# Aleph-Alpha/magma

Measured on NVIDIA H100. Metric: image-caption samples/sec (fwd+bwd), higher is better.
Workload: dtype bf16

## Files before the change

include/magma_b200.h:

```cpp
#ifndef MAGMA_B200_H_
#define MAGMA_B200_H_

#include <stddef.h>
#include <stdint.h>

#ifdef __cplusplus
extern "C" {
#endif

#define MB200_VERSION 100

enum {
  MB200_OK = 0,
  MB200_E_SHAPE = -1,
  MB200_E_DTYPE = -2,
  MB200_E_ALIGN = -3,
  MB200_E_ARCH = -4,
  MB200_E_CUDA = -5,
  MB200_E_NCCL = -6,
  MB200_E_ARG = -7
};

enum { MB200_BF16 = 0, MB200_F32 = 1 };

enum {
  MB200_ACT_NONE = 0,
  MB200_ACT_GELU_NEW = 1,
  MB200_ACT_QUICK_GELU = 2,
  MB200_ACT_RELU = 3,
  MB200_ACT_RELU_POST = 4
};
enum {
  MB200_DACT_NONE = 0,
  MB200_DACT_GELU_NEW = 1,
  MB200_DACT_RELU = 3
};

int mb200_version(void);
const char* mb200_last_error(void);
int mb200_check_device(void);
int mb200_set_gemm_sm_limit(int n_sms);
int mb200_set_optimizer_grid(int n_blocks);
long long mb200_launch_count(void);
int mb200_prof_enable(int on);
int mb200_prof_read(double* gemm_ms, double* gemm_flops, double* gemm_bytes, long long* gemm_launches);

typedef struct {
  const void* ptr;
  int64_t ld;
  int64_t bs0, bs1;
  int32_t mn_major;
  int32_t static_data;
} mb200_operand;

typedef struct {
  int32_t M, N, K;
  int32_t nb0, nb1;
  int32_t c_dtype;
  mb200_operand A, B;
  void* C;
  int64_t ldc, c_bs0, c_bs1;
  float alpha;
  int32_t act;
  int32_t dact;
  int32_t accumulate;
  const void* bias;
  void* aux_out;
  const void* aux_in;
  const void* res1;
  const void* res2;
  int64_t ld_res;
  int32_t force_bn;
  int32_t generic_epilogue;
  int32_t rope_mode;
  const void* rope_tab;
  int32_t rope_S, rope_hd, rope_rot, rope_ncols;
  void* splitk_ws;
  int64_t splitk_ws_bytes;
} mb200_gemm_args;

int mb200_gemm(const mb200_gemm_args* args, void* stream);


int mb200_layernorm_fwd(const void* x, int64_t ldx, const void* gamma, const void* beta, void* y, int64_t ldy,
                        float* mean, float* rstd, int32_t rows, int32_t d, float eps, void* stream);
int mb200_layernorm_bwd(const void* dy, int64_t lddy, const void* x, int64_t ldx, const void* gamma,
                        const float* mean, const float* rstd, const void* res, int64_t ldres, void* dx, int64_t lddx,
                        int32_t rows, int32_t d, void* stream);
int mb200_layernorm_param_grad(const void* dy, int64_t lddy, const void* x, int64_t ldx, const float* mean,
                               const float* rstd, float* dgamma, float* dbeta, int32_t rows, int32_t d,
                               int32_t accumulate, void* stream);
int mb200_layernorm_param_grad_rows(const void* dy, int64_t lddy, const void* x, int64_t ldx, const float* mean,
                                    const float* rstd, float* dgamma, float* dbeta, int32_t rows, int32_t d,
                                    int32_t accumulate, void* stream);
int mb200_rope(void* qkv, int64_t ld, int32_t rows, int32_t S, int32_t H, int32_t hd, int32_t rot, int32_t pos0,
               int32_t inverse, void* stream);
int mb200_rope_table(float* tab, int32_t S, int32_t rot, int32_t pos0, void* stream);
int mb200_softmax_fwd(const float* s, int64_t lds, int64_t s_bs, void* p, int64_t ldp, int64_t p_bs, int32_t nz,
                      int32_t Sq, int32_t Sk, float scale, int32_t causal, int32_t koff, void* stream);
int mb200_softmax_bwd(const float* dp, int64_t lddp, int64_t dp_bs, const void* p, int64_t ldp, int64_t p_bs,
                      void* ds, int64_t ldds, int64_t ds_bs, int32_t nz, int32_t Sq, int32_t Sk, float scale,
                      void* stream);
int mb200_build_labels(const int64_t* captions, int64_t ldc, int64_t* labels, int32_t B, int32_t S, int32_t L,
                       int64_t eos, void* stream);
int mb200_embed_assemble(const int64_t* captions, int64_t ldc, const void* wte, const void* prefix, int32_t L,
                         void* x, int32_t B, int32_t S, int32_t d, int32_t vocab, void* stream);
int mb200_embed_gather(const int64_t* ids, const void* wte, void* out, int32_t n, int32_t d, int32_t vocab,
                       void* stream);
int mb200_cross_entropy(const void* logits, int64_t ldv, const int64_t* labels, int32_t B, int32_t S, int32_t V,
                        float* row_loss, int32_t* n_valid, float* loss, void* dlogits, float grad_scale,
                        void* stream);
int mb200_colsum(const void* x, int64_t ldx, int32_t rows, int32_t cols, float* out, int32_t accumulate,
                 void* stream);
int mb200_dropout_fwd(const void* x, void* y, uint8_t* mask, int64_t n, float p, uint64_t seed, void* stream);
int mb200_dropout_apply(const void* x, const uint8_t* mask, void* y, int64_t n, float p, void* stream);
int mb200_patchify(const void* img, void* patches, int64_t ldp, int32_t B, int32_t R, int32_t P, void* stream);
int mb200_vit_assemble(void* x, const void* pe, const void* cls, const void* pos, int32_t B, int32_t T, int32_t w,
                       void* stream);
int mb200_nchw_to_nhwc8(const void* src, void* dst, int32_t B, int32_t C, int32_t H, int32_t W, void* stream);
int mb200_im2col3x3(const void* src, void* dst, int32_t B, int32_t H, int32_t W, int32_t C, int32_t stride,
                    void* stream);
int mb200_avgpool_nhwc(const void* src, void* dst, int32_t B, int32_t H, int32_t W, int32_t C, int32_t k, void* stream);
int mb200_col_moments(const void* u, int64_t ldu, const void* v, int64_t ldv, const void* mask, int64_t ldm, int32_t rows,
                      int32_t cols, float* out1, float* out2, void* stream);
int mb200_channel_affine(const void* x1, const float* a1, const void* x2, const float* a2, const float* c0,
                         const void* mask, const void* res, int32_t relu, void* y, int64_t rows, int32_t C, void* stream);
int mb200_bn_finalize_fwd(const float* s1, const float* s2, const float* gamma, const float* beta, int64_t rows, float eps,
                          float momentum, float* running_mean, float* running_var, float* mean, float* rstd, float* scale,
                          float* shift, int32_t C, void* stream);
int mb200_bn_bwd_coeffs(const float* s1, const float* t, const float* mean, const float* rstd, const float* gamma,
                        int64_t rows, float* dgamma, float* dbeta, int32_t accumulate, float* A, float* Bc, float* Cc,
                        int32_t C, void* stream);
int mb200_col2im3x3(const void* dcols, void* dx, int32_t B, int32_t H, int32_t W, int32_t C, int32_t stride, void* stream);
int mb200_avgpool_nhwc_bwd(const void* dy, void* dx, int32_t B, int32_t H, int32_t W, int32_t C, int32_t k, void* stream);
int mb200_argmax(const void* x, int64_t ldx, int32_t rows, int32_t V, int64_t* out, void* stream);
int mb200_sample(const void* logits, int32_t dtype, int64_t ld, int32_t rows, int32_t V, float temperature,
                 int32_t top_k, float top_p, uint64_t seed, uint64_t offset, int64_t* tokens, uint8_t* keep_mask,
                 void* stream);
int mb200_add(const void* a, const void* b, const void* c, void* y, int64_t n, void* stream);
int mb200_peer_reduce_bcast(void* const* bufs, int32_t world, int64_t offset, int64_t n, int32_t max_blocks,
                            void* stream);

int mb200_sumsq(const float* x, int64_t n, float* out, void* stream);
int mb200_adamw_step(float* master, float* grad, float* exp_avg, float* exp_avg_sq, void* shadow_bf16, int64_t n,
                     float lr, float beta1, float beta2, float eps, float weight_decay, float grad_scale,
                     const float* gnorm_sq, float max_norm, int32_t step, int32_t zero_grad, void* stream);
int mb200_cast_f32_to_bf16(const float* src, void* dst, int64_t n, void* stream);
int mb200_cast_bf16_to_f32(const void* src, float* dst, int64_t n, void* stream);

enum { MB200_ADAPTER_NONE = 0, MB200_ADAPTER_NORMAL = 1, MB200_ADAPTER_PARALLEL = 2 };

typedef struct {
  const void *ln1_g, *ln1_b;
  const void* w_qkv;
  const void* b_qkv;
  const void* w_out;
  const void* b_out;
  const void *ln2_g, *ln2_b;
  const void* w_fc;
  const void* b_fc;
  const void* w_proj;
  const void* b_proj;
} mb200_vit_layer;

// ... 143 lines not shown
```

magma_b200/_lib.py:

```python
import ctypes
import os

_HERE = os.path.dirname(os.path.abspath(__file__))
LIB_PATH = os.path.join(_HERE, "lib", "libmagma_b200.so")

_lib = None


class MB200Error(RuntimeError):
    pass


class Operand(ctypes.Structure):
    _fields_ = [
        ("ptr", ctypes.c_void_p),
        ("ld", ctypes.c_int64),
        ("bs0", ctypes.c_int64),
        ("bs1", ctypes.c_int64),
        ("mn_major", ctypes.c_int32),
        ("static_data", ctypes.c_int32),
    ]


class GemmArgs(ctypes.Structure):
# ... 59 lines not shown
        (n, ctypes.c_void_p)
        for n in (
            "ln1_g", "ln1_b", "w_qkv", "b_qkv", "w_out", "b_out", "ln2_g", "ln2_b", "w_fc", "b_fc", "w_proj", "b_proj",
        )
    ]


class VitModelC(ctypes.Structure):
    _fields_ = [
        ("n_layer", ctypes.c_int32),
        ("width", ctypes.c_int32),
        ("n_head", ctypes.c_int32),
        ("patch", ctypes.c_int32),
        ("image", ctypes.c_int32),
        ("mlp", ctypes.c_int32),
        ("out_dim", ctypes.c_int32),
        ("_pad", ctypes.c_int32),
        ("w_conv", ctypes.c_void_p),
        ("ld_conv", ctypes.c_int64),
        ("cls", ctypes.c_void_p),
        ("pos", ctypes.c_void_p),
        ("ln_pre_g", ctypes.c_void_p),
        ("ln_pre_b", ctypes.c_void_p),
        ("ln_post_g", ctypes.c_void_p),
        ("ln_post_b", ctypes.c_void_p),
        ("proj_t", ctypes.c_void_p),
        ("layers", ctypes.POINTER(VitLayerC)),
    ]


class AdapterExC(ctypes.Structure):
    _fields_ = [(n, ctypes.c_void_p) for n in ("wd", "bd", "wu", "bu", "ln_g", "ln_b", "scale", "g_wd", "g_bd", "g_wu",
                                               "g_bu", "g_ln_g", "g_ln_b", "g_scale")]


class GptjLayerExC(ctypes.Structure):
    _fields_ = [
        (n, ctypes.c_void_p)
        for n in ("ln1_g", "ln1_b", "w_qkv", "w_out", "w_fc_in", "b_fc_in", "w_fc_out", "b_fc_out")
    ] + [("mlp_ad", AdapterExC), ("attn_ad", AdapterExC)]


class GptjModelExC(ctypes.Structure):
    _fields_ = [
        ("n_layer", ctypes.c_int32),
        ("d", ctypes.c_int32),
        ("n_head", ctypes.c_int32),
        ("rotary_dim", ctypes.c_int32),
        ("vocab", ctypes.c_int32),
        ("d_ff", ctypes.c_int32),
        ("mlp_adapter", ctypes.c_int32),
        ("mlp_adapter_r", ctypes.c_int32),
        ("attn_adapter", ctypes.c_int32),
        ("attn_adapter_r", ctypes.c_int32),
        ("ln_eps", ctypes.c_float),
        ("adapter_act", ctypes.c_int32),
        ("layers", ctypes.POINTER(GptjLayerExC)),
        ("lnf_g", ctypes.c_void_p),
        ("lnf_b", ctypes.c_void_p),
        ("w_lm", ctypes.c_void_p),
        ("b_lm", ctypes.c_void_p),
    ]


class VitLayerGradsC(ctypes.Structure):
    _fields_ = list(VitLayerC._fields_)


class VitGradsC(ctypes.Structure):
    _fields_ = [(n, ctypes.c_void_p) for n in ("w_conv", "cls", "pos", "ln_pre_g", "ln_pre_b", "ln_post_g",
                                               "ln_post_b", "proj")] + [("layers", ctypes.POINTER(VitLayerGradsC))]


def _setup_signatures(L):
    L.mb200_vit_workspace_bytes.restype = ctypes.c_size_t
    L.mb200_vit_train_workspace_bytes.restype = ctypes.c_size_t
    L.mb200_gptj_sched_workspace_bytes.restype = ctypes.c_size_t
    L.mb200_gptj_sched_infer_workspace_bytes.restype = ctypes.c_size_t
    L.mb200_gptj_sched_recompute_workspace_bytes.restype = ctypes.c_size_t
    L.mb200_launch_count.restype = ctypes.c_longlong


EXPORTED_SYMBOLS = [
    "mb200_version", "mb200_last_error", "mb200_check_device", "mb200_gemm",
    "mb200_launch_count", "mb200_prof_enable", "mb200_prof_read",
    "mb200_layernorm_fwd", "mb200_layernorm_bwd", "mb200_layernorm_param_grad", "mb200_rope", "mb200_rope_table",
    "mb200_softmax_fwd", "mb200_softmax_bwd", "mb200_build_labels", "mb200_embed_assemble", "mb200_embed_gather",
    "mb200_cross_entropy", "mb200_colsum", "mb200_dropout_fwd", "mb200_dropout_apply", "mb200_patchify",
    "mb200_nchw_to_nhwc8", "mb200_im2col3x3", "mb200_avgpool_nhwc",
    "mb200_vit_assemble", "mb200_argmax", "mb200_sample", "mb200_add", "mb200_peer_reduce_bcast", "mb200_sumsq", "mb200_adamw_step",
    "mb200_cast_f32_to_bf16", "mb200_cast_bf16_to_f32",
    "mb200_vit_workspace_bytes", "mb200_vit_forward", "mb200_attn_decode", "mb200_attn_fwd_tile", "mb200_attn_fwd_flash",
    "mb200_attn_bwd_tile",
    "mb200_vit_train_workspace_bytes", "mb200_vit_forward_train", "mb200_vit_backward", "mb200_quick_gelu_bwd",
    "mb200_layernorm_param_grad_rows", "mb200_set_gemm_sm_limit", "mb200_set_optimizer_grid", "mb200_scale_add", "mb200_dot",
    "mb200_gptj_sched_workspace_bytes", "mb200_gptj_sched_forward", "mb200_gptj_sched_backward",
    "mb200_col_moments", "mb200_channel_affine", "mb200_col2im3x3", "mb200_avgpool_nhwc_bwd",
    "mb200_kv_append", "mb200_gptj_sched_infer_workspace_bytes", "mb200_gptj_sched_infer",
    "mb200_gptj_sched_backward_range", "mb200_bn_finalize_fwd", "mb200_bn_bwd_coeffs",
    "mb200_gptj_sched_decode_step", "mb200_decode_embed", "mb200_decode_advance", "mb200_rope_table_dev",
    "mb200_attn_decode_dev", "mb200_gptj_sched_recompute_workspace_bytes", "mb200_gptj_sched_forward_recompute",
    "mb200_gptj_sched_backward_range_recompute",
]
```

magma_b200/csrc/gemm.cu:

```cuda
#include <mutex>
#include <stdlib.h>

#include "gemm_common.cuh"

namespace mb200 {

template <bool kOn>
struct EpiMaps {
  CUtensorMap m[3];
};
template <>
struct EpiMaps<false> {};

template <int BN, bool A_MN, bool B_MN, bool EPI_TMA, uint32_t FORM = EF_RUNTIME>
__global__ void __launch_bounds__(kThreads, 1)
gemm_wgmma_kernel(const __grid_constant__ CUtensorMap tmA, const __grid_constant__ CUtensorMap tmB,
                  const __grid_constant__ EpiMaps<EPI_TMA> tmE, const __grid_constant__ GemmKernelParams p) {
  using C_ = Cfg<BN>;
  constexpr int kStages = C_::kStages;

  extern __shared__ uint8_t smem_raw[];
  uint8_t* smem = smem_raw + ((1024u - (smem_u32(smem_raw) & 1023u)) & 1023u);
  uint8_t* smem_a = smem;
  uint8_t* smem_b = smem + kStages * C_::kABytes;
// ... 171 lines not shown
  cuuint32_t estr[4] = {1, 1, 1, 1};
  if (!op.mn_major) {
    dims[0] = (cuuint64_t)K;
    dims[1] = (cuuint64_t)rows;
    box[0] = BK;
    box[1] = (cuuint32_t)box_rows;
  } else {
    dims[0] = (cuuint64_t)rows;
    dims[1] = (cuuint64_t)K;
    box[0] = 64;
    box[1] = BK;
  }
  dims[2] = (cuuint64_t)nb0;
  dims[3] = (cuuint64_t)nb1;
  box[2] = 1;
  box[3] = 1;
  strides[0] = (cuuint64_t)op.ld * 2;
  strides[1] = (cuuint64_t)(nb0 > 1 ? op.bs0 : op.ld) * 2;
  strides[2] = (cuuint64_t)(nb1 > 1 ? op.bs1 : op.ld) * 2;
  CUresult r = enc(out, CU_TENSOR_MAP_DATA_TYPE_BFLOAT16, 4, const_cast<void*>(op.ptr), dims, strides, box, estr,
                   CU_TENSOR_MAP_INTERLEAVE_NONE, CU_TENSOR_MAP_SWIZZLE_128B, CU_TENSOR_MAP_L2_PROMOTION_L2_256B,
                   CU_TENSOR_MAP_FLOAT_OOB_FILL_NONE);
  MB_REQUIRE(r == CUDA_SUCCESS, MB200_E_CUDA,
             "cuTensorMapEncodeTiled failed (%d): dims=(%llu,%llu,%llu,%llu) strides=(%llu,%llu,%llu) box=(%u,%u)",
             (int)r, (unsigned long long)dims[0], (unsigned long long)dims[1], (unsigned long long)dims[2],
             (unsigned long long)dims[3], (unsigned long long)strides[0], (unsigned long long)strides[1],
             (unsigned long long)strides[2], box[0], box[1]);
  return 0;
}

template <int BN, bool A_MN, bool B_MN, bool EPI_TMA, uint32_t FORM = EF_RUNTIME>
static int launch_gemm(const CUtensorMap& tmA, const CUtensorMap& tmB, const EpiMaps<true>& tmE,
                       const GemmKernelParams& kp, cudaStream_t stream) {
  auto kern = gemm_wgmma_kernel<BN, A_MN, B_MN, EPI_TMA, FORM>;
  static bool attr_set = false;
  if (!attr_set) {
    MB_CUDA(cudaFuncSetAttribute(kern, cudaFuncAttributeMaxDynamicSharedMemorySize, Cfg<BN>::kSmemBytes));
    attr_set = true;
  }
  const long long items = (long long)kp.total_tiles * kp.split_k;
  int grid = items < gemm_sms() ? (int)items : gemm_sms();
  {
    const double nb = (double)kp.total_tiles / ((double)kp.tiles_m * kp.tiles_n);
    const double flops = 2.0 * kp.M * (double)kp.N * kp.K * nb;
    const double bytes = nb * (2.0 * ((double)kp.M * kp.K + (double)kp.N * kp.K) + (kp.c_f32 ? 4.0 : 2.0) * kp.M * kp.N);
    GemmProfScope prof(stream, flops, bytes);
    if constexpr (EPI_TMA)
      MB_CUDA(launch_pdl(kern, dim3(grid), dim3(kThreads), Cfg<BN>::kSmemBytes, stream, tmA, tmB, tmE, kp));
    else
      MB_CUDA(launch_pdl(kern, dim3(grid), dim3(kThreads), Cfg<BN>::kSmemBytes, stream, tmA, tmB, EpiMaps<false>{}, kp));
  }
  count_launch();
  MB_CUDA(cudaGetLastError());
  return 0;
}

template <int BN, bool EPI_TMA>
static int dispatch_major(bool a_mn, bool b_mn, const CUtensorMap& tmA, const CUtensorMap& tmB,
                          const EpiMaps<true>& tmE, const GemmKernelParams& kp, cudaStream_t s) {
  if (!a_mn && !b_mn) return launch_gemm<BN, false, false, EPI_TMA>(tmA, tmB, tmE, kp, s);
  if (!a_mn && b_mn) return launch_gemm<BN, false, true, EPI_TMA>(tmA, tmB, tmE, kp, s);
  if (a_mn && !b_mn) return launch_gemm<BN, true, false, EPI_TMA>(tmA, tmB, tmE, kp, s);
  return launch_gemm<BN, true, true, EPI_TMA>(tmA, tmB, tmE, kp, s);
}

static int dispatch_bn(int bn, bool a_mn, bool b_mn, const CUtensorMap& tmA, const CUtensorMap& tmB,
                       const EpiMaps<true>& tmE, const GemmKernelParams& kp, cudaStream_t s) {
  const bool epi = kp.epi_in != 0;
  switch (bn) {
    case 64:
      return epi ? dispatch_major<64, true>(a_mn, b_mn, tmA, tmB, tmE, kp, s)
                 : dispatch_major<64, false>(a_mn, b_mn, tmA, tmB, tmE, kp, s);
    case 128:
      return epi ? dispatch_major<128, true>(a_mn, b_mn, tmA, tmB, tmE, kp, s)
                 : dispatch_major<128, false>(a_mn, b_mn, tmA, tmB, tmE, kp, s);
    default:
      return epi ? dispatch_major<256, true>(a_mn, b_mn, tmA, tmB, tmE, kp, s)
                 : dispatch_major<256, false>(a_mn, b_mn, tmA, tmB, tmE, kp, s);
  }
}

template <uint32_t F, bool A_MN, bool B_MN>
static bool launch_form(uint32_t form, bool a_mn, bool b_mn, const CUtensorMap& tmA, const CUtensorMap& tmB,
                        const EpiMaps<true>& tmE, const GemmKernelParams& kp, cudaStream_t s, int* rc) {
  if (form != F || a_mn != A_MN || b_mn != B_MN) return false;
  *rc = launch_gemm<256, A_MN, B_MN, EpiForm<F>::kInputs != 0, F>(tmA, tmB, tmE, kp, s);
  return true;
}
static bool dispatch_form(uint32_t form, bool a_mn, bool b_mn, const CUtensorMap& tmA, const CUtensorMap& tmB,
                          const EpiMaps<true>& tmE, const GemmKernelParams& kp, cudaStream_t s, int* rc) {
#define MB_FORM(F, A_MN, B_MN) launch_form<(F), A_MN, B_MN>(form, a_mn, b_mn, tmA, tmB, tmE, kp, s, rc)
  return MB_FORM(EF_ROPE, false, false) ||
         MB_FORM(EF_RES1, false, false) ||
         MB_FORM(EF_BIAS | EF_GELU | EF_AUX_OUT, false, false) ||
         MB_FORM(EF_BIAS, false, false) ||
         MB_FORM(EF_BIAS | EF_RES1 | EF_RES2, false, false) ||
         MB_FORM(EF_DGELU, false, true) ||
         MB_FORM(0u, false, true) ||
         MB_FORM(EF_RES1, false, true) ||
         MB_FORM(EF_F32, true, true);
#undef MB_FORM
}

static uint32_t epi_form(const mb200_gemm_args* a, const GemmKernelParams& kp, int bn) {
  if (a->generic_epilogue || bn != 256) return EF_RUNTIME;
  if ((a->act != MB200_ACT_NONE && a->act != MB200_ACT_GELU_NEW) ||
      (a->dact != MB200_DACT_NONE && a->dact != MB200_DACT_GELU_NEW))
    return EF_RUNTIME;
  if (((reinterpret_cast<uintptr_t>(a->bias) | reinterpret_cast<uintptr_t>(a->aux_out)) & 7) != 0) return EF_RUNTIME;
  const uint32_t f = (a->bias ? EF_BIAS : 0u) | (kp.rope_mode ? EF_ROPE : 0u) | (a->aux_out ? EF_AUX_OUT : 0u) |
                     (a->act ? EF_GELU : 0u) | (a->dact ? EF_DGELU : 0u) | (a->res1 ? EF_RES1 : 0u) |
                     (a->res2 ? EF_RES2 : 0u) | (kp.c_f32 ? EF_F32 : 0u);
  const int inputs = (a->dact != 0) + (a->res1 != nullptr) + (a->res2 != nullptr);
  return kp.epi_in == inputs ? f : EF_RUNTIME;
}

static int make_epi_maps(EpiMaps<true>* maps, GemmKernelParams* kp, const mb200_gemm_args* a) {
  const void* ptr[3];
  long long ld[3];
  int n = 0;
  if (a->dact) {
    ptr[n] = a->aux_in;
    ld[n++] = a->ldc;
  }
  if (a->res1) {
    ptr[n] = a->res1;
    ld[n++] = a->ld_res;
  }
  if (a->res2) {
    ptr[n] = a->res2;
    ld[n++] = a->ld_res;
  }
  bool ok = (a->nb0 == 1 || a->c_bs0 % 8 == 0) && (a->nb1 == 1 || a->c_bs1 % 8 == 0);
  for (int i = 0; i < n; ++i) ok = ok && (reinterpret_cast<uintptr_t>(ptr[i]) & 15) == 0 && ld[i] % 8 == 0;
  if (n == 0 || !ok) return 0;
  for (int i = 0; i < n; ++i) {
    mb200_operand op;
    memset(&op, 0, sizeof(op));
    op.ptr = ptr[i];
    op.ld = ld[i];
    op.bs0 = a->c_bs0;
    op.bs1 = a->c_bs1;
    const int rc = make_operand_map(&maps->m[i], op, a->M, a->N, a->nb0, a->nb1, BM);
    if (rc) return rc;
  }
  kp->epi_in = n;
  return 0;
}

static int pick_bn(int M, int N, int batches) {
  if (N <= 64) return 64;
  const int tiles_m = (M + BM - 1) / BM;
  const int sms = num_sms();
  double best = 1e300;
  int best_bn = 256;
  const int cands[3] = {256, 128, 64};
  const double tile_cost[3] = {1.0, 0.55, 0.3};
  for (int i = 0; i < 3; ++i) {
    const int bn = cands[i];
    if (bn > 64 && N <= bn / 2) continue;
    const long long t = (long long)tiles_m * ((N + bn - 1) / bn) * batches;
    const long long waves = (t + sms - 1) / sms;
    const double cost = (double)waves * tile_cost[i];
    if (cost < best - 1e-12) {
      best = cost;
      best_bn = bn;
    }
  }
  return best_bn;
}

struct SmallPlan {
  int bn, split;
};
static SmallPlan plan_small_m(int N, int K, int M, size_t ws_bytes) {
  const int sms = num_sms();
  const int num_kb = (K + BK - 1) / BK;
  const double kHbmRate = 3.35e12, kItem = 4e-6, kFinalize = 4e-6;
  SmallPlan best{64, 1};
  double best_t = 1e300;
  const int cands[3] = {256, 128, 64};
  for (int i = 0; i < 3; ++i) {
    const int bn = cands[i];
    if (bn > 64 && N <= bn / 2) continue;
    const int tiles = (N + bn - 1) / bn;
    for (int split = 1; split <= 16; ++split) {
      if (split > 1) {
        if (num_kb / split < 8) break;
        if ((size_t)split * M * ((N + 3) / 4 * 4) * sizeof(float) > ws_bytes) break;
      }
      const int kb_per = (num_kb + split - 1) / split;
      const int eff_split = (num_kb + kb_per - 1) / kb_per;
      const long long items = (long long)tiles * eff_split;
      const long long waves = (items + sms - 1) / sms;
      const double active = (double)(items < sms ? items : sms);
      const double sm_rate = bn == 64 ? 40e9 : 50e9;
      const double rate = sm_rate < kHbmRate / active ? sm_rate : kHbmRate / active;
      const double t = kItem + waves * ((double)kb_per * bn * BK * 2 / rate) + (eff_split > 1 ? kFinalize : 0.0);
      if (t < best_t - 1e-12) {
        best_t = t;
        best = SmallPlan{bn, eff_split};
      }
    }
  }
  return best;
}

int gemm_impl(const mb200_gemm_args* a, cudaStream_t stream) {
  MB_REQUIRE(a != nullptr, MB200_E_ARG, "null gemm args");
  MB_REQUIRE(a->M > 0 && a->N > 0 && a->K > 0 && a->nb0 > 0 && a->nb1 > 0, MB200_E_SHAPE,
             "gemm: bad shape M=%d N=%d K=%d nb=(%d,%d)", a->M, a->N, a->K, a->nb0, a->nb1);
  MB_REQUIRE(a->c_dtype == MB200_BF16 || a->c_dtype == MB200_F32, MB200_E_DTYPE, "gemm: bad c_dtype %d", a->c_dtype);
  MB_REQUIRE(!(a->accumulate && a->c_dtype != MB200_F32), MB200_E_DTYPE, "gemm: accumulate needs f32 output");
  MB_REQUIRE(!(a->dact && !a->aux_in), MB200_E_ARG, "gemm: dact needs aux_in");
  const int celt = a->c_dtype == MB200_F32 ? 4 : 8;
  MB_REQUIRE((reinterpret_cast<uintptr_t>(a->C) & 15) == 0 && a->ldc % celt == 0, MB200_E_ALIGN,
             "gemm: C must be 16B aligned with ldc multiple of %d", celt);
  MB_REQUIRE((a->nb0 == 1 || a->c_bs0 % celt == 0) && (a->nb1 == 1 || a->c_bs1 % celt == 0), MB200_E_ALIGN,
             "gemm: C batch strides must be multiples of %d elements", celt);
  if (a->res1 || a->res2) MB_REQUIRE(a->ld_res % 8 == 0, MB200_E_ALIGN, "gemm: ld_res must be a multiple of 8");
  if (a->aux_in || a->aux_out)
    MB_REQUIRE(a->ldc % 8 == 0, MB200_E_ALIGN, "gemm: aux tensors share ldc, which must be a multiple of 8");
  int rc = check_arch();
  if (rc) return rc;

  int bn = a->force_bn ? a->force_bn : pick_bn(a->M, a->N, a->nb0 * a->nb1);
  MB_REQUIRE(bn == 64 || bn == 128 || bn == 256, MB200_E_ARG, "gemm: force_bn must be 64, 128 or 256");

  CUtensorMap tmA, tmB;
  EpiMaps<true> tmE;
  memset(&tmE, 0, sizeof(tmE));
  const bool small_m = a->M <= 32 && a->A.mn_major == 0 && a->nb0 * a->nb1 == 1 && a->c_dtype == MB200_BF16;
  int plan_split = 1;
  if (small_m && !a->force_bn) {
    const SmallPlan pl = plan_small_m(a->N, a->K, a->M, a->splitk_ws ? (size_t)a->splitk_ws_bytes : 0);
    bn = pl.bn;
    plan_split = pl.split;
  }
  rc = make_operand_map(&tmA, a->A, a->M, a->K, a->nb0, a->nb1, BM);
  if (rc) return rc;

  GemmKernelParams kp;
  memset(&kp, 0, sizeof(kp));
  kp.M = a->M;
  kp.N = a->N;
  kp.K = a->K;
  kp.nb0 = a->nb0;
  kp.tiles_m = (a->M + BM - 1) / BM;
  kp.C = a->C;
  kp.ldc = a->ldc;
  kp.c_bs0 = a->c_bs0;
  kp.c_bs1 = a->c_bs1;
  kp.alpha = a->alpha;
  kp.act = a->act;
  kp.dact = a->dact;
  kp.accumulate = a->accumulate;
  kp.bias = reinterpret_cast<const bf16*>(a->bias);
  kp.aux_out = reinterpret_cast<bf16*>(a->aux_out);
  kp.aux_in = reinterpret_cast<const bf16*>(a->aux_in);
  kp.res1 = reinterpret_cast<const bf16*>(a->res1);
  kp.res2 = reinterpret_cast<const bf16*>(a->res2);
  kp.ld_res = a->ld_res;
  kp.epi_kind = EK_GENERIC;
  kp.c_f32 = a->c_dtype == MB200_F32 ? 1 : 0;
  kp.rope_tab = reinterpret_cast<const float2*>(a->rope_tab);
  kp.rope_mode = a->rope_tab ? a->rope_mode : 0;
  kp.rope_S = a->rope_S;
  kp.rope_hd = a->rope_hd;
  kp.rope_rot = a->rope_rot;
  kp.rope_ncols = a->rope_ncols;
  if (kp.rope_mode != 0)
    MB_REQUIRE(a->rope_S > 0 && a->rope_hd > 0 && a->rope_rot % 4 == 0 && a->rope_rot <= a->rope_hd &&
                   a->rope_hd % 4 == 0 && a->rope_ncols % 4 == 0,
               MB200_E_ARG, "gemm: bad rope epilogue parameters");

  const bool amn = a->A.mn_major != 0, bmn = a->B.mn_major != 0;
  kp.split_k = 1;
  kp.kb_per_split = (a->K + BK - 1) / BK;
  const bool split_mid = !small_m && a->splitk_ws && a->M <= 128 && a->nb0 * a->nb1 == 1 && a->K >= 8192 &&
                         a->N <= 8192 && !a->force_bn;
  const int bn_few = a->N >= 256 ? 256 : (a->N > 64 ? 128 : 64);
  const int tiles_m = kp.tiles_m;
  const bool split_few = !small_m && !split_mid && a->splitk_ws && a->M > 128 && a->nb0 * a->nb1 == 1 &&
                         a->K >= 2048 && !a->force_bn && 2 * tiles_m * ((a->N + bn_few - 1) / bn_few) <= num_sms();
  if (plan_split > 1 || split_mid || split_few) {
    const int bn_s = small_m ? bn : bn_few;
    const int tiles = (a->N + bn_s - 1) / bn_s;
    const int num_kb = (a->K + BK - 1) / BK;
    int split = plan_split;
    if (split_mid || split_few) {
      split = num_sms() / (tiles * tiles_m);
      if (split > num_kb / 4) split = num_kb / 4;
    }
    const long long ld_ws = (a->N + 3) / 4 * 4;
    while (split > 1 && (size_t)split * a->M * ld_ws * sizeof(float) > (size_t)a->splitk_ws_bytes) --split;
    if (split > 1) {
      const int kb_per = (num_kb + split - 1) / split;
      split = (num_kb + kb_per - 1) / kb_per;
      bn = bn_s;
      rc = make_operand_map(&tmB, a->B, a->N, a->K, a->nb0, a->nb1, bn);
      if (rc) return rc;
      kp.tiles_n = tiles;
      kp.total_tiles = tiles_m * tiles;
      kp.split_k = split;
      kp.kb_per_split = kb_per;
      kp.splitk_ws = reinterpret_cast<float*>(a->splitk_ws);
      kp.ld_ws = ld_ws;
      GemmKernelParams kg = kp;
      kg.epi_kind = EK_SPLITK;
      rc = dispatch_bn(bn, amn, bmn, tmA, tmB, tmE, kg, stream);
      if (rc) return rc;
      const long long n4 = (long long)a->M * ((a->N + 3) / 4);
      const int fgrid = (int)((n4 + 255) / 256 > 2048 ? 2048 : (n4 + 255) / 256);
      kp.alpha = 1.f;
      MB_CUDA(launch_pdl(splitk_finalize_kernel, dim3(fgrid), dim3(256), 0, stream, kp));
      count_launch();
      return 0;
    }
  }
  rc = make_operand_map(&tmB, a->B, a->N, a->K, a->nb0, a->nb1, bn);
  if (rc) return rc;
  kp.tiles_n = (a->N + bn - 1) / bn;
  kp.total_tiles = tiles_m * kp.tiles_n * a->nb0 * a->nb1;
  rc = make_epi_maps(&tmE, &kp, a);
  if (rc) return rc;
  if (dispatch_form(epi_form(a, kp, bn), amn, bmn, tmA, tmB, tmE, kp, stream, &rc)) return rc;
  return dispatch_bn(bn, amn, bmn, tmA, tmB, tmE, kp, stream);
}

}

extern "C" int mb200_gemm(const mb200_gemm_args* args, void* stream) {
  return mb200::gemm_impl(args, reinterpret_cast<cudaStream_t>(stream));
}
```

magma_b200/csrc/gemm_common.cuh:

```cuda
#pragma once
#include <type_traits>

#include "common.cuh"

namespace mb200 {

static constexpr int BM = 128;
static constexpr int BK = 64;
static constexpr int WG_K = 16;
static constexpr int kThreads = 384;
static constexpr int kEpiCols = 64;
static constexpr int kEpiBytes = BM * kEpiCols * 4;
static constexpr int kEpiBoxBytes = BM * kEpiCols * 2;
static constexpr int kSmemBudget = 192 * 1024;

template <int BN>
struct Cfg {
  static constexpr int kABytes = BM * BK * 2;
  static constexpr int kBBytes = BN * BK * 2;
  static constexpr int kStageBytes = kABytes + kBBytes;
  static constexpr int kStagesRaw = kSmemBudget / kStageBytes;
  static constexpr int kStages = kStagesRaw > 8 ? 8 : kStagesRaw;
  static constexpr int kSmemBytes = kStages * kStageBytes + kEpiBytes + 1024  + 256 ;
  static_assert(kSmemBytes <= 227 * 1024, "GEMM shared memory exceeds the sm_90 per-block limit");
  static constexpr int kEpiBoxesPerStage = 1 + kBBytes / kEpiBoxBytes;
  static_assert(kABytes == kEpiBoxBytes && kEpiBoxesPerStage * kEpiBoxBytes <= kStageBytes, "epilogue box layout");
  static_assert(3 * (BN / kEpiCols) <= kStages * kEpiBoxesPerStage, "epilogue inputs exceed the operand ring");
};

struct GemmKernelParams {
  int M, N, K;
  int nb0;
  int tiles_m, tiles_n, total_tiles;
  void* C;
  long long ldc, c_bs0, c_bs1;
  float alpha;
  int act, dact, accumulate;
  const bf16* bias;
  bf16* aux_out;
  const bf16* aux_in;
  const bf16* res1;
  const bf16* res2;
  long long ld_res;
  int epi_in;
  const float2* rope_tab;
  int rope_mode;
  int rope_S, rope_hd, rope_rot, rope_ncols;
  int epi_kind;
  int c_f32;
  int split_k, kb_per_split;
  float* splitk_ws;
  long long ld_ws;
};

__device__ __forceinline__ float2 bf16x2_to_f32(uint32_t u) {
  return __bfloat1622float2(*reinterpret_cast<const __nv_bfloat162*>(&u));
}
__device__ __forceinline__ uint32_t f32x2_to_bf16(float a, float b) {
  __nv_bfloat162 h = __floats2bfloat162_rn(a, b);
  return *reinterpret_cast<uint32_t*>(&h);
}

template <bool kVec = false>
__device__ __forceinline__ void ld_bf16x4(const bf16* src, int n, float (&v)[4]) {
  if (kVec || (n == 4 && (reinterpret_cast<uintptr_t>(src) & 7) == 0)) {
    uint32_t u0, u1;
    asm volatile("ld.global.nc.v2.u32 {%0, %1}, [%2];" : "=r"(u0), "=r"(u1) : "l"(src));
    const float2 a = bf16x2_to_f32(u0), b = bf16x2_to_f32(u1);
    v[0] = a.x;
    v[1] = a.y;
    v[2] = b.x;
    v[3] = b.y;
  } else {
#pragma unroll
    for (int e = 0; e < 4; ++e) v[e] = e < n ? __bfloat162float(src[e]) : 0.f;
  }
}
template <bool kVec = false>
__device__ __forceinline__ void st_bf16x4(bf16* dst, int n, const float (&v)[4]) {
  if (kVec || (n == 4 && (reinterpret_cast<uintptr_t>(dst) & 7) == 0)) {
    *reinterpret_cast<uint2*>(dst) = make_uint2(f32x2_to_bf16(v[0], v[1]), f32x2_to_bf16(v[2], v[3]));
  } else {
#pragma unroll
    for (int e = 0; e < 4; ++e)
      if (e < n) dst[e] = __float2bfloat16(v[e]);
  }
}

__device__ __forceinline__ void named_bar_sync(int id, int nthreads) {
  asm volatile("bar.sync %0, %1;" ::"r"(id), "r"(nthreads) : "memory");
}

enum { EK_GENERIC = 0, EK_SPLITK };

enum : uint32_t {
  EF_BIAS = 1,
  EF_ROPE = 2,
  EF_AUX_OUT = 4,
  EF_GELU = 8,
  EF_DGELU = 16,
  EF_RES1 = 32,
  EF_RES2 = 64,
  EF_F32 = 128,
  EF_RUNTIME = 1u << 31
};

template <uint32_t F>
struct EpiForm {
  static constexpr bool kRuntime = F == EF_RUNTIME;
  static constexpr int kInputs = kRuntime ? 0 : ((F & EF_DGELU) != 0) + ((F & EF_RES1) != 0) + ((F & EF_RES2) != 0);
  static constexpr int kRows = kRuntime ? 1 : 8;
  using P = GemmKernelParams;
  static __device__ __forceinline__ bool bias(const P& p) { return kRuntime ? p.bias != nullptr : (F & EF_BIAS) != 0; }
  static __device__ __forceinline__ bool rope(const P& p) { return kRuntime ? p.rope_mode != 0 : (F & EF_ROPE) != 0; }
  static __device__ __forceinline__ bool aux_out(const P& p) {
    return kRuntime ? p.aux_out != nullptr : (F & EF_AUX_OUT) != 0;
  }
  static __device__ __forceinline__ int act(const P& p) {
    return kRuntime ? p.act : (F & EF_GELU) ? MB200_ACT_GELU_NEW : MB200_ACT_NONE;
  }
  static __device__ __forceinline__ int dact(const P& p) {
    return kRuntime ? p.dact : (F & EF_DGELU) ? MB200_DACT_GELU_NEW : MB200_DACT_NONE;
  }
  static __device__ __forceinline__ bool res1(const P& p) { return kRuntime ? p.res1 != nullptr : (F & EF_RES1) != 0; }
  static __device__ __forceinline__ bool res2(const P& p) { return kRuntime ? p.res2 != nullptr : (F & EF_RES2) != 0; }
  static __device__ __forceinline__ bool c_f32(const P& p) { return kRuntime ? p.c_f32 != 0 : (F & EF_F32) != 0; }
  static __device__ __forceinline__ bool accumulate(const P& p) { return (kRuntime || (F & EF_F32)) && p.accumulate; }
  static __device__ __forceinline__ bool splitk(const P& p) { return kRuntime && p.epi_kind == EK_SPLITK; }
};

struct EpiIn {
  float aux[4], res1[4], res2[4];
};

template <class Form>
__device__ __forceinline__ void epi_load_inputs(const GemmKernelParams& p, long long boff, int row, int col,
                                                EpiIn& in) {
  const int n = min(4, p.N - col);
  if (Form::dact(p)) ld_bf16x4(p.aux_in + boff + (long long)row * p.ldc + col, n, in.aux);
  const long long roff = boff + (long long)row * p.ld_res + col;
  if (Form::res1(p)) ld_bf16x4(p.res1 + roff, n, in.res1);
  if (Form::res2(p)) ld_bf16x4(p.res2 + roff, n, in.res2);
}

__device__ __forceinline__ void ld_smem_bf16x4(const uint8_t* src, float (&v)[4]) {
  const uint2 u = *reinterpret_cast<const uint2*>(src);
  const float2 a = bf16x2_to_f32(u.x), b = bf16x2_to_f32(u.y);
  v[0] = a.x;
  v[1] = a.y;
  v[2] = b.x;
  v[3] = b.y;
}

template <class Form, bool kVec = false>
__device__ __forceinline__ void epi_store4(const GemmKernelParams& p, long long boff, int row, int col, float (&v)[4],
                                           const float (&bias)[4], const EpiIn& in) {
  const int n = min(4, p.N - col);
  if (Form::bias(p)) {
#pragma unroll
    for (int e = 0; e < 4; ++e) v[e] += bias[e];
  }
  if (Form::rope(p) && col < p.rope_ncols) {
    const int dim = col % p.rope_hd;
    if (dim < p.rope_rot) {
      const float2* tp = p.rope_tab + (long long)(row % p.rope_S) * (p.rope_rot >> 1) + (dim >> 1);
      const float2 cs0 = __ldg(tp), cs1 = __ldg(tp + 1);
      const float sg = p.rope_mode > 0 ? 1.f : -1.f;
      const float a0 = v[0], a1 = v[1], a2 = v[2], a3 = v[3];
      v[0] = a0 * cs0.x - a1 * cs0.y * sg;
      v[1] = a1 * cs0.x + a0 * cs0.y * sg;
      v[2] = a2 * cs1.x - a3 * cs1.y * sg;
      v[3] = a3 * cs1.x + a2 * cs1.y * sg;
    }
  }
  const long long coff = boff + (long long)row * p.ldc + col;
  if (Form::aux_out(p)) st_bf16x4<kVec>(p.aux_out + coff, n, v);
#pragma unroll
  for (int e = 0; e < 4; ++e) {
    if (Form::act(p) == MB200_ACT_GELU_NEW) v[e] = gelu_new_f(v[e]);
    else if (Form::act(p) == MB200_ACT_QUICK_GELU) v[e] = quick_gelu_f(v[e]);
    else if (Form::act(p) == MB200_ACT_RELU) v[e] = fmaxf(v[e], 0.f);
  }
  if (Form::dact(p)) {
#pragma unroll
    for (int e = 0; e < 4; ++e)
      v[e] = Form::dact(p) == MB200_DACT_GELU_NEW ? v[e] * gelu_new_grad_f(in.aux[e]) : (in.aux[e] > 0.f ? v[e] : 0.f);
  }
  if (Form::res1(p)) {
#pragma unroll
    for (int e = 0; e < 4; ++e) v[e] += in.res1[e];
  }
  if (Form::res2(p)) {
#pragma unroll
    for (int e = 0; e < 4; ++e) v[e] += in.res2[e];
  }
  if (Form::act(p) == MB200_ACT_RELU_POST) {
#pragma unroll
    for (int e = 0; e < 4; ++e) v[e] = fmaxf(v[e], 0.f);
  }
  if (Form::c_f32(p)) {
    float* dst = reinterpret_cast<float*>(p.C) + coff;
    if (kVec || n == 4) {
// ... 180 lines not shown
```

magma_b200/ops.py:

```python
import ctypes

import torch

from . import _lib
from ._lib import GemmArgs, check, lib

ACT_NONE, ACT_GELU_NEW, ACT_QUICK_GELU, ACT_RELU, ACT_RELU_POST = 0, 1, 2, 3, 4
DACT_NONE, DACT_GELU_NEW, DACT_RELU = 0, 1, 3


def _stream():
    return ctypes.c_void_p(torch.cuda.current_stream().cuda_stream)


def _ptr(t):
    return ctypes.c_void_p(t.data_ptr()) if t is not None else None


def _mat_meta(t, name):
    if t.dim() < 2 or t.dim() > 4:
        raise ValueError(f"{name}: expected 2-4 dims, got {t.dim()}")
    if t.stride(-1) != 1 and t.shape[-1] != 1:
        raise ValueError(f"{name}: innermost stride must be 1, got {t.stride()}")
    rows, cols = t.shape[-2], t.shape[-1]
# ... 14 lines not shown
    b_mn=False,
    out_dtype=torch.bfloat16,
    alpha=1.0,
    bias=None,
    act=ACT_NONE,
    aux_out=None,
    aux_in=None,
    dact=DACT_NONE,
    res1=None,
    res2=None,
    accumulate=False,
    force_bn=0,
    generic_epilogue=False,
    rope_tab=None,
    rope_mode=0,
    rope_S=0,
    rope_hd=0,
    rope_rot=0,
    rope_ncols=0,
    splitk_ws=None,
    b_static=False,
):
    if A.dtype != torch.bfloat16 or B.dtype != torch.bfloat16:
        raise TypeError("gemm operands must be bf16")
    ra, ca, lda, anb0, anb1, abs0, abs1 = _mat_meta(A, "A")
    rb, cb, ldb, bnb0, bnb1, bbs0, bbs1 = _mat_meta(B, "B")
    M, K = (ca, ra) if a_mn else (ra, ca)
    N, Kb = (cb, rb) if b_mn else (rb, cb)
    if K != Kb:
        raise ValueError(f"gemm K mismatch: {K} vs {Kb}")
    nb0, nb1 = max(anb0, bnb0), max(anb1, bnb1)
    if (anb0, anb1) != (nb0, nb1) or (bnb0, bnb1) != (nb0, nb1):
        raise ValueError("gemm: A and B must have identical batch dims")
    if out is None:
        shape = ([nb1] if A.dim() >= 4 else []) + ([nb0] if A.dim() >= 3 else []) + [M, N]
        out = torch.empty(shape, dtype=out_dtype, device=A.device)
    rc_, cc, ldc, cnb0, cnb1, cbs0, cbs1 = _mat_meta(out, "out")
    if (rc_, cc) != (M, N) or (cnb0, cnb1) != (nb0, nb1):
        raise ValueError(f"gemm: out shape {tuple(out.shape)} does not match M={M} N={N} batch=({nb1},{nb0})")
    g = GemmArgs()
    g.M, g.N, g.K, g.nb0, g.nb1 = M, N, K, nb0, nb1
    g.c_dtype = 1 if out.dtype == torch.float32 else 0
    if out.dtype not in (torch.float32, torch.bfloat16):
        raise TypeError("gemm out must be bf16 or f32")
    g.A.ptr, g.A.ld, g.A.bs0, g.A.bs1, g.A.mn_major = A.data_ptr(), lda, abs0, abs1, int(a_mn)
    g.B.ptr, g.B.ld, g.B.bs0, g.B.bs1, g.B.mn_major = B.data_ptr(), ldb, bbs0, bbs1, int(b_mn)
    g.B.static_data = int(bool(b_static))
    g.C, g.ldc, g.c_bs0, g.c_bs1 = out.data_ptr(), ldc, cbs0, cbs1
    g.alpha, g.act, g.dact, g.accumulate = float(alpha), int(act), int(dact), int(bool(accumulate))
    for name, t in (("bias", bias), ("aux_out", aux_out), ("aux_in", aux_in), ("res1", res1), ("res2", res2)):
        if t is not None:
            if t.dtype != torch.bfloat16:
                raise TypeError(f"gemm {name} must be bf16")
            setattr(g, name, t.data_ptr())
    if bias is not None and (tuple(bias.shape) != (N,) or (N > 1 and bias.stride(0) != 1)):
        raise ValueError(f"gemm bias must be a contiguous [N={N}] vector, got shape {tuple(bias.shape)}")
    for name, t in (("aux_out", aux_out), ("aux_in", aux_in), ("res1", res1), ("res2", res2)):
        if t is not None and tuple(t.shape) != tuple(out.shape):
            raise ValueError(f"gemm {name} shape {tuple(t.shape)} must equal out's {tuple(out.shape)}")
    for name, t in (("aux_out", aux_out), ("aux_in", aux_in)):
        if t is not None and _mat_meta(t, name)[2:] != (ldc, cnb0, cnb1, cbs0, cbs1):
            raise ValueError(f"gemm {name} must share out's strides")
    ld_res = 0
    for name, t in (("res1", res1), ("res2", res2)):
        if t is not None:
            m = _mat_meta(t, name)
            if (cnb0 > 1 and m[5] != cbs0) or (cnb1 > 1 and m[6] != cbs1):
                raise ValueError(f"gemm {name} must share out's batch strides (its row stride may differ)")
            if ld_res and m[2] != ld_res:
                raise ValueError("res1/res2 must share a row stride")
            ld_res = m[2]
    g.ld_res = ld_res
    g.force_bn = force_bn
    g.generic_epilogue = int(bool(generic_epilogue))
    if rope_tab is not None and rope_mode:
        g.rope_tab, g.rope_mode = rope_tab.data_ptr(), int(rope_mode)
        g.rope_S, g.rope_hd, g.rope_rot, g.rope_ncols = int(rope_S), int(rope_hd), int(rope_rot), int(rope_ncols)
    if splitk_ws is not None:
        g.splitk_ws, g.splitk_ws_bytes = splitk_ws.data_ptr(), splitk_ws.numel() * splitk_ws.element_size()
    check(lib().mb200_gemm(ctypes.byref(g), _stream()))
    return out


def _rows(t):
    d = t.shape[-1]
    if t.dim() == 1:
        return 1, d, d
    t2 = t.reshape(-1, d) if t.is_contiguous() else None
    if t2 is not None:
        return t2.shape[0], d, d
    if t.dim() == 2:
        return t.shape[0], d, t.stride(0)
    raise ValueError("non-contiguous >2-D tensor: pass a 2-D view with an explicit row stride")


def layernorm_fwd(x, gamma, beta, eps=1e-5, save_stats=True, out=None):
    rows, d, ldx = _rows(x)
    y = torch.empty(x.shape, dtype=torch.bfloat16, device=x.device) if out is None else out
    mean = torch.empty(rows, dtype=torch.float32, device=x.device) if save_stats else None
    rstd = torch.empty(rows, dtype=torch.float32, device=x.device) if save_stats else None
    check(lib().mb200_layernorm_fwd(_ptr(x), ctypes.c_int64(ldx), _ptr(gamma), _ptr(beta), _ptr(y),
                                    ctypes.c_int64(_rows(y)[2]), _ptr(mean), _ptr(rstd), rows, d,
                                    ctypes.c_float(eps), _stream()))
    return y, mean, rstd


def layernorm_bwd(dy, x, gamma, mean, rstd, res=None, out=None):
    rows, d, ldx = _rows(x)
    dx = torch.empty(x.shape, dtype=torch.bfloat16, device=x.device) if out is None else out
    check(lib().mb200_layernorm_bwd(_ptr(dy), ctypes.c_int64(_rows(dy)[2]), _ptr(x), ctypes.c_int64(ldx), _ptr(gamma),
                                    _ptr(mean), _ptr(rstd), _ptr(res), ctypes.c_int64(_rows(res)[2] if res is not None else 0),
                                    _ptr(dx), ctypes.c_int64(_rows(dx)[2]), rows, d, _stream()))
    return dx


def layernorm_param_grad(dy, x, mean, rstd, dgamma, dbeta, accumulate=False):
    rows, d, ldx = _rows(x)
    check(lib().mb200_layernorm_param_grad(_ptr(dy), ctypes.c_int64(_rows(dy)[2]), _ptr(x), ctypes.c_int64(ldx),
                                           _ptr(mean), _ptr(rstd), _ptr(dgamma), _ptr(dbeta), rows, d,
                                           int(accumulate), _stream()))


def layernorm_param_grad_rows(dy, x, mean, rstd, dgamma, dbeta, accumulate=False):
    rows, d, ldx = _rows(x)
    check(lib().mb200_layernorm_param_grad_rows(_ptr(dy), ctypes.c_int64(_rows(dy)[2]), _ptr(x), ctypes.c_int64(ldx),
                                                _ptr(mean), _ptr(rstd), _ptr(dgamma), _ptr(dbeta), rows, d,
                                                int(accumulate), _stream()))


def quick_gelu_bwd(dy, pre, out=None):
    out = torch.empty_like(dy) if out is None else out
    check(lib().mb200_quick_gelu_bwd(_ptr(dy), _ptr(pre), _ptr(out), ctypes.c_int64(dy.numel()), _stream()))
    return out


def rope_(qkv, S, H, hd, rot, pos0=0, inverse=False):
    rows = qkv.shape[0]
    check(lib().mb200_rope(_ptr(qkv), ctypes.c_int64(qkv.stride(0)), rows, S, H, hd, rot, pos0, int(inverse), _stream()))
    return qkv


def rope_table(S, rot, pos0=0, device=None):
    tab = torch.empty(S, rot // 2, 2, dtype=torch.float32, device=device or torch.device("cuda"))
    check(lib().mb200_rope_table(_ptr(tab), S, rot, pos0, _stream()))
    return tab


def softmax_fwd(s, scale, causal, koff=0, out=None):
    nz, Sq, Sk = s.shape
    lds = s.stride(1)
    p = torch.zeros(nz, Sq, lds, dtype=torch.bfloat16, device=s.device)[..., :Sk] if out is None else out
    _batched_out(p, "out", (nz, Sq, Sk))
    check(lib().mb200_softmax_fwd(_ptr(s), ctypes.c_int64(lds), ctypes.c_int64(s.stride(0)), _ptr(p),
                                  ctypes.c_int64(p.stride(1)), ctypes.c_int64(p.stride(0)), nz, Sq, Sk,
                                  ctypes.c_float(scale), int(causal), koff, _stream()))
    return p


def _batched_out(t, name, shape):
    if t.dtype != torch.bfloat16 or tuple(t.shape) != shape or (shape[-1] > 1 and t.stride(-1) != 1):
        raise ValueError(f"{name} must be a bf16 {list(shape)} view with unit column stride, got {t.dtype} "
                         f"{tuple(t.shape)} strides {t.stride()}")


def softmax_bwd(dp, p, scale, out=None):
    nz, Sq, Sk = dp.shape
# ... 354 lines not shown
```

Baseline: 153.3.

## Add compiled epilogue forms and make tile-width choice epilogue-aware

Adds two compile-time epilogue specialisations (bias+residual and bias+quick-GELU) so those GEMMs avoid the runtime-branching epilogue. The tile-N heuristic now takes K and whether a compiled form exists, weighing mainloop work per tile against a fixed epilogue cost so the 256-wide specialised path is preferred when it applies. A thread-local record of the last chosen plan and a query function are exposed for inspection. This adds more template instantiations to compile, and the new cost constants may pick worse tiles for some shapes.

```diff
diff --git a/include/magma_b200.h b/include/magma_b200.h
--- a/include/magma_b200.h
+++ b/include/magma_b200.h
@@ -80,6 +80,7 @@
 } mb200_gemm_args;
 
 int mb200_gemm(const mb200_gemm_args* args, void* stream);
+int mb200_gemm_last_plan(int32_t* bn, int32_t* split_k);
 
 
 int mb200_layernorm_fwd(const void* x, int64_t ldx, const void* gamma, const void* beta, void* y, int64_t ldy,
diff --git a/magma_b200/_lib.py b/magma_b200/_lib.py
--- a/magma_b200/_lib.py
+++ b/magma_b200/_lib.py
@@ -165,7 +165,7 @@
 
 
 EXPORTED_SYMBOLS = [
-    "mb200_version", "mb200_last_error", "mb200_check_device", "mb200_gemm",
+    "mb200_version", "mb200_last_error", "mb200_check_device", "mb200_gemm", "mb200_gemm_last_plan",
     "mb200_launch_count", "mb200_prof_enable", "mb200_prof_read",
     "mb200_layernorm_fwd", "mb200_layernorm_bwd", "mb200_layernorm_param_grad", "mb200_rope", "mb200_rope_table",
     "mb200_softmax_fwd", "mb200_softmax_bwd", "mb200_build_labels", "mb200_embed_assemble", "mb200_embed_gather",
diff --git a/magma_b200/csrc/gemm.cu b/magma_b200/csrc/gemm.cu
--- a/magma_b200/csrc/gemm.cu
+++ b/magma_b200/csrc/gemm.cu
@@ -277,19 +277,21 @@
 
 template <uint32_t F, bool A_MN, bool B_MN>
 static bool launch_form(uint32_t form, bool a_mn, bool b_mn, const CUtensorMap& tmA, const CUtensorMap& tmB,
-                        const EpiMaps<true>& tmE, const GemmKernelParams& kp, cudaStream_t s, int* rc) {
+                        const EpiMaps<true>& tmE, const GemmKernelParams* kp, cudaStream_t s, int* rc) {
   if (form != F || a_mn != A_MN || b_mn != B_MN) return false;
-  *rc = launch_gemm<256, A_MN, B_MN, EpiForm<F>::kInputs != 0, F>(tmA, tmB, tmE, kp, s);
+  if (kp) *rc = launch_gemm<256, A_MN, B_MN, EpiForm<F>::kInputs != 0, F>(tmA, tmB, tmE, *kp, s);
   return true;
 }
 static bool dispatch_form(uint32_t form, bool a_mn, bool b_mn, const CUtensorMap& tmA, const CUtensorMap& tmB,
-                          const EpiMaps<true>& tmE, const GemmKernelParams& kp, cudaStream_t s, int* rc) {
+                          const EpiMaps<true>& tmE, const GemmKernelParams* kp, cudaStream_t s, int* rc) {
 #define MB_FORM(F, A_MN, B_MN) launch_form<(F), A_MN, B_MN>(form, a_mn, b_mn, tmA, tmB, tmE, kp, s, rc)
   return MB_FORM(EF_ROPE, false, false) ||
          MB_FORM(EF_RES1, false, false) ||
          MB_FORM(EF_BIAS | EF_GELU | EF_AUX_OUT, false, false) ||
          MB_FORM(EF_BIAS, false, false) ||
          MB_FORM(EF_BIAS | EF_RES1 | EF_RES2, false, false) ||
+         MB_FORM(EF_BIAS | EF_RES1, false, false) ||
+         MB_FORM(EF_BIAS | EF_QGELU, false, false) ||
          MB_FORM(EF_DGELU, false, true) ||
          MB_FORM(0u, false, true) ||
          MB_FORM(EF_RES1, false, true) ||
@@ -297,17 +299,22 @@
 #undef MB_FORM
 }
 
-static uint32_t epi_form(const mb200_gemm_args* a, const GemmKernelParams& kp, int bn) {
-  if (a->generic_epilogue || bn != 256) return EF_RUNTIME;
-  if ((a->act != MB200_ACT_NONE && a->act != MB200_ACT_GELU_NEW) ||
+static uint32_t epi_form(const mb200_gemm_args* a, const GemmKernelParams& kp) {
+  if ((a->act != MB200_ACT_NONE && a->act != MB200_ACT_GELU_NEW && a->act != MB200_ACT_QUICK_GELU) ||
       (a->dact != MB200_DACT_NONE && a->dact != MB200_DACT_GELU_NEW))
     return EF_RUNTIME;
   if (((reinterpret_cast<uintptr_t>(a->bias) | reinterpret_cast<uintptr_t>(a->aux_out)) & 7) != 0) return EF_RUNTIME;
   const uint32_t f = (a->bias ? EF_BIAS : 0u) | (kp.rope_mode ? EF_ROPE : 0u) | (a->aux_out ? EF_AUX_OUT : 0u) |
-                     (a->act ? EF_GELU : 0u) | (a->dact ? EF_DGELU : 0u) | (a->res1 ? EF_RES1 : 0u) |
-                     (a->res2 ? EF_RES2 : 0u) | (kp.c_f32 ? EF_F32 : 0u);
+                     (a->act == MB200_ACT_GELU_NEW ? EF_GELU : 0u) | (a->act == MB200_ACT_QUICK_GELU ? EF_QGELU : 0u) |
+                     (a->dact ? EF_DGELU : 0u) | (a->res1 ? EF_RES1 : 0u) | (a->res2 ? EF_RES2 : 0u) |
+                     (kp.c_f32 ? EF_F32 : 0u);
   const int inputs = (a->dact != 0) + (a->res1 != nullptr) + (a->res2 != nullptr);
-  return kp.epi_in == inputs ? f : EF_RUNTIME;
+  if (kp.epi_in != inputs) return EF_RUNTIME;
+  CUtensorMap unused;
+  EpiMaps<true> unused_e;
+  return dispatch_form(f, a->A.mn_major != 0, a->B.mn_major != 0, unused, unused, unused_e, nullptr, 0, nullptr)
+             ? f
+             : EF_RUNTIME;
 }
 
 static int make_epi_maps(EpiMaps<true>* maps, GemmKernelParams* kp, const mb200_gemm_args* a) {
@@ -343,20 +350,23 @@
   return 0;
 }
 
-static int pick_bn(int M, int N, int batches) {
+static int pick_bn(int M, int N, int K, int batches, bool compiled_form) {
   if (N <= 64) return 64;
   const int tiles_m = (M + BM - 1) / BM;
+  const int num_kb = (K + BK - 1) / BK;
   const int sms = num_sms();
+  const bool weigh_epi = compiled_form && tiles_m >= 8;
+  const double kTile[3] = {1.0, 0.55, 0.3}, kEpiRuntime = 32.0, kEpiForm = 8.0;
+  const int cands[3] = {256, 128, 64};
   double best = 1e300;
   int best_bn = 256;
-  const int cands[3] = {256, 128, 64};
-  const double tile_cost[3] = {1.0, 0.55, 0.3};
   for (int i = 0; i < 3; ++i) {
     const int bn = cands[i];
     if (bn > 64 && N <= bn / 2) continue;
     const long long t = (long long)tiles_m * ((N + bn - 1) / bn) * batches;
     const long long waves = (t + sms - 1) / sms;
-    const double cost = (double)waves * tile_cost[i];
+    const double epi = bn == 256 ? kEpiForm : kEpiRuntime * bn / 256;
+    const double cost = (double)waves * (weigh_epi ? num_kb * kTile[i] + epi : kTile[i]);
     if (cost < best - 1e-12) {
       best = cost;
       best_bn = bn;
@@ -364,6 +374,8 @@
   }
   return best_bn;
 }
+
+static thread_local int t_plan[2] = {0, 0};
 
 struct SmallPlan {
   int bn, split;
@@ -419,8 +431,8 @@
   int rc = check_arch();
   if (rc) return rc;
 
-  int bn = a->force_bn ? a->force_bn : pick_bn(a->M, a->N, a->nb0 * a->nb1);
-  MB_REQUIRE(bn == 64 || bn == 128 || bn == 256, MB200_E_ARG, "gemm: force_bn must be 64, 128 or 256");
+  int bn = a->force_bn;
+  MB_REQUIRE(bn == 0 || bn == 64 || bn == 128 || bn == 256, MB200_E_ARG, "gemm: force_bn must be 64, 128 or 256");
 
   CUtensorMap tmA, tmB;
   EpiMaps<true> tmE;
@@ -510,17 +522,27 @@
       kp.alpha = 1.f;
       MB_CUDA(launch_pdl(splitk_finalize_kernel, dim3(fgrid), dim3(256), 0, stream, kp));
       count_launch();
+      t_plan[0] = bn;
+      t_plan[1] = split;
       return 0;
     }
   }
+  rc = make_epi_maps(&tmE, &kp, a);
+  if (rc) return rc;
+  const uint32_t form = epi_form(a, kp);
+  if (bn == 0) bn = pick_bn(a->M, a->N, a->K, a->nb0 * a->nb1, form != EF_RUNTIME);
   rc = make_operand_map(&tmB, a->B, a->N, a->K, a->nb0, a->nb1, bn);
   if (rc) return rc;
   kp.tiles_n = (a->N + bn - 1) / bn;
   kp.total_tiles = tiles_m * kp.tiles_n * a->nb0 * a->nb1;
-  rc = make_epi_maps(&tmE, &kp, a);
-  if (rc) return rc;
-  if (dispatch_form(epi_form(a, kp, bn), amn, bmn, tmA, tmB, tmE, kp, stream, &rc)) return rc;
-  return dispatch_bn(bn, amn, bmn, tmA, tmB, tmE, kp, stream);
+  if (!(!a->generic_epilogue && bn == 256 && form != EF_RUNTIME &&
+        dispatch_form(form, amn, bmn, tmA, tmB, tmE, &kp, stream, &rc)))
+    rc = dispatch_bn(bn, amn, bmn, tmA, tmB, tmE, kp, stream);
+  if (rc == 0) {
+    t_plan[0] = bn;
+    t_plan[1] = 1;
+  }
+  return rc;
 }
 
 }
@@ -528,3 +550,9 @@
 extern "C" int mb200_gemm(const mb200_gemm_args* args, void* stream) {
   return mb200::gemm_impl(args, reinterpret_cast<cudaStream_t>(stream));
 }
+
+extern "C" int mb200_gemm_last_plan(int32_t* bn, int32_t* split_k) {
+  if (bn) *bn = mb200::t_plan[0];
+  if (split_k) *split_k = mb200::t_plan[1];
+  return 0;
+}
diff --git a/magma_b200/csrc/gemm_common.cuh b/magma_b200/csrc/gemm_common.cuh
--- a/magma_b200/csrc/gemm_common.cuh
+++ b/magma_b200/csrc/gemm_common.cuh
@@ -102,6 +102,7 @@
   EF_RES1 = 32,
   EF_RES2 = 64,
   EF_F32 = 128,
+  EF_QGELU = 256,
   EF_RUNTIME = 1u << 31
 };
 
@@ -117,7 +118,10 @@
     return kRuntime ? p.aux_out != nullptr : (F & EF_AUX_OUT) != 0;
   }
   static __device__ __forceinline__ int act(const P& p) {
-    return kRuntime ? p.act : (F & EF_GELU) ? MB200_ACT_GELU_NEW : MB200_ACT_NONE;
+    return kRuntime ? p.act
+           : (F & EF_GELU) ? MB200_ACT_GELU_NEW
+           : (F & EF_QGELU) ? MB200_ACT_QUICK_GELU
+                            : MB200_ACT_NONE;
   }
   static __device__ __forceinline__ int dact(const P& p) {
     return kRuntime ? p.dact : (F & EF_DGELU) ? MB200_DACT_GELU_NEW : MB200_DACT_NONE;
diff --git a/magma_b200/ops.py b/magma_b200/ops.py
--- a/magma_b200/ops.py
+++ b/magma_b200/ops.py
@@ -120,6 +120,12 @@
     return out
 
 
+def gemm_last_plan():
+    v = [ctypes.c_int32() for _ in range(2)]
+    lib().mb200_gemm_last_plan(*[ctypes.byref(x) for x in v])
+    return tuple(x.value for x in v)
+
+
 def _rows(t):
     d = t.shape[-1]
     if t.dim() == 1:
```

After: 158.1 (median of 6 runs). 3.1% higher.
